# yh-jun/SNR-Aligned_diffSE

Measured on AMD Instinct MI355X. Metric: utterances/sec (4 s @16 kHz, N=30 PC steps) at 1/2/4/8 MI355X; PESQ delta vs ref, higher is better.
Workload: dtype fp16; 1 GPU; C2: B=32 4 s/16 kHz clips per GPU, N=30 PC steps (reverse_diffusion + ald, 60 NFE/utt), OUVE SDE, NCSN++ nf=128, fp16; global_batch=32, per_gpu_batch=32, seq_len=512, parallelism=dp1 (utterance sharding)

## Files before the change

### snr-aligned_diffse_amd/csrc/conv.hip

```cpp
#include "conv_common.h"

#include <algorithm>
#include <type_traits>

using namespace snrse_conv;

namespace {

template <int NWM, int BN>
SNRSE_DEV void block_stats_flush(const ConvParams& p, const float* red, int blk_b, int blk_n0) {
  asm volatile("s_waitcnt lgkmcnt(0)" ::: "memory");
  __builtin_amdgcn_s_barrier();
  const int slot = blockIdx.x & (SNRSE_STAT_SLOTS - 1);
  for (int t = threadIdx.x; t < 2 * BN; t += blockDim.x) {
    float a = 0.f;
#pragma unroll
    for (int w = 0; w < NWM; ++w) a += red[w * 2 * BN + t];
    if (blk_n0 + (t >> 1) < p.Cout)
      unsafeAtomicAdd(&p.stats[stat_idx(blk_b, slot, blk_n0 + (t >> 1), p.Cout) + (t & 1)], (double)a);
  }
}

template <typename TO, int NWM, int BN, bool DEFER = false, int LA = 8>
SNRSE_DEV void epilogue_lds(const ConvParams& p, const f32x4 (&acc)[4][4], int mb, int nb, int lane, float* stage,
// ... 953 lines not shown
                                                 (float*)(smem + 8 * (64 * 68 * 4)), wr, bb, n0, p.W - TW);
}

template <int BM, int BN, typename T, typename TO>
__global__ __launch_bounds__(512) void conv_glds_kernel(ConvParams p) {
  constexpr int WM = BM / 64, WN = BN / 64;
  static_assert(WM * WN == 8, "8 waves");
  constexpr int FM = 4, FN = 4, TM = 64, TN = 64;
  constexpr int STAGES = 3;
  constexpr int A_BYTES = BM * 128, B_BYTES = BN * 128, STAGE = A_BYTES + B_BYTES;
  constexpr int AJ = BM / 64, BJ = BN / 64;
  constexpr int KT = 64;
  extern __shared__ __attribute__((aligned(16))) char smem[];

  const int tid = threadIdx.x, lane = tid & 63;
  const int wid = __builtin_amdgcn_readfirstlane(tid >> 6);
  const int wm = wid / WN, wn = wid % WN;
  const int wg = xcd_block_id(blockIdx.x, gridDim.x);
  const int ks = wg % p.ksplit, tl = wg / p.ksplit;
  const int m0 = (tl / p.ntn) * BM;
  const int n0 = (tl % p.ntn) * BN;

  const int HW = p.H * p.W;
  const int Cin = p.C0 + p.C1;
  const int cblocks = Cin / KT;
  const int nk0 = p.ksize * p.ksize * cblocks;
  const int Csc_all = p.Csc + p.Csc1;
  const int nk = nk0 + (p.sc_src ? Csc_all / KT : 0);
  const int K1 = p.ksize * p.ksize * Cin;
  const int half = p.ksize >> 1;
  const int slot = lane & 7;

  int a_pix[AJ], a_h[AJ], a_w[AJ], a_ch[AJ];
  bool a_ok[AJ];
#pragma unroll
  for (int j = 0; j < AJ; ++j) {
    const int row = (wid * AJ + j) * 8 + (lane >> 3);
    const int m = m0 + row;
    a_ok[j] = m < p.M;
    const int mm = a_ok[j] ? m : 0;
    const int b = mm / HW, rem = mm - b * HW;
    a_h[j] = rem / p.W;
    a_w[j] = rem - a_h[j] * p.W;
    a_pix[j] = mm;
    a_ch[j] = slot ^ (row & 7);
  }

#define SNRSE_ISSUE(KT_, STAGE_)                                                                      \
  do {                                                                                              \
    const int kt_ = (KT_);                                                                          \
    char* sa_ = smem + (STAGE_) * STAGE;                                                            \
    char* sb_ = sa_ + A_BYTES;                                                                      \
    int cs_, cc_, dy_, dx_, wld_, koff_;                                                            \
    const void* abase_;                                                                             \
    long long abytes_;                                                                              \
    const void* wbase_;                                                                             \
    long long wbytes_;                                                                              \
    if (kt_ < nk0) {                                                                                \
      const int tap_ = kt_ / cblocks;                                                               \
      const int c_ = (kt_ - tap_ * cblocks) * KT;                                                   \
      dy_ = tap_ / p.ksize - half;                                                                  \
      dx_ = tap_ - (tap_ / p.ksize) * p.ksize - half;                                               \
      const bool u1_ = c_ >= p.C0;                                                                  \
      abase_ = u1_ ? p.src1 : p.src0;                                                               \
      abytes_ = u1_ ? p.bytes1 : p.bytes0;                                                          \
      cs_ = u1_ ? p.C1 : p.C0;                                                                      \
      cc_ = u1_ ? c_ - p.C0 : c_;                                                                   \
      wbase_ = p.wgt;                                                                               \
      wbytes_ = p.wbytes;                                                                           \
      wld_ = K1;                                                                                    \
      koff_ = tap_ * Cin + c_;                                                                      \
    } else {                                                                                        \
      const int c_ = (kt_ - nk0) * KT;                                                              \
      const bool u1_ = c_ >= p.Csc;                                                                 \
      abase_ = u1_ ? p.sc_src1 : p.sc_src;                                                          \
      abytes_ = u1_ ? p.sc_bytes1 : p.sc_bytes0;                                                    \
      cs_ = u1_ ? p.Csc1 : p.Csc;                                                                   \
      cc_ = u1_ ? c_ - p.Csc : c_;                                                                  \
      dy_ = 0;                                                                                      \
      dx_ = 0;                                                                                      \
      wbase_ = p.sc_wgt;                                                                            \
      wbytes_ = p.sc_wbytes;                                                                        \
      wld_ = Csc_all;                                                                               \
      koff_ = c_;                                                                                   \
    }                                                                                               \
    const __amdgpu_buffer_rsrc_t ra_ = make_rsrc(abase_, abytes_);                                  \
    const __amdgpu_buffer_rsrc_t rb_ = make_rsrc(wbase_, wbytes_);                                  \
    const int shift_ = dy_ * p.W + dx_;                                                             \
    _Pragma("unroll") for (int j = 0; j < AJ; ++j) {                                                \
      const int hh_ = a_h[j] + dy_, ww_ = a_w[j] + dx_;                                             \
      const bool ok_ = a_ok[j] && hh_ >= 0 && hh_ < p.H && ww_ >= 0 && ww_ < p.W;                   \
      const unsigned voff_ =                                                                        \
          ok_ ? (unsigned)(((a_pix[j] + shift_) * cs_ + cc_ + a_ch[j] * 8) * 2) : 0x80000000u;      \
      __builtin_amdgcn_raw_ptr_buffer_load_lds(                                                     \
          ra_, (__attribute__((address_space(3))) void*)(sa_ + (wid * AJ + j) * 1024), 16, voff_, 0, 0, 0); \
    }                                                                                               \
    _Pragma("unroll") for (int j = 0; j < BJ; ++j) {                                                \
      const int row_ = (wid * BJ + j) * 8 + (lane >> 3);                                            \
      const int chk_ = slot ^ (row_ & 7);                                                           \
      const unsigned voff_ = (unsigned)(((n0 + row_) * wld_ + koff_ + chk_ * 8) * 2);               \
      __builtin_amdgcn_raw_ptr_buffer_load_lds(                                                     \
          rb_, (__attribute__((address_space(3))) void*)(sb_ + (wid * BJ + j) * 1024), 16, voff_, 0, 0, 0); \
    }                                                                                               \
  } while (0)

  f32x4 acc[FM][FN];
#pragma unroll
  for (int i = 0; i < FM; ++i)
#pragma unroll
    for (int j = 0; j < FN; ++j) acc[i][j] = f32x4{0.f, 0.f, 0.f, 0.f};

  const int kb = (int)((long long)ks * nk / p.ksplit), ke = (int)((long long)(ks + 1) * nk / p.ksplit);
  SNRSE_ISSUE(kb, 0);
  if (ke - kb > 1) SNRSE_ISSUE(kb + 1, 1);
  const int lrow = lane & 15, lg = lane >> 4;
  int stage = 0;
  for (int kt = kb; kt < ke; ++kt) {
    if (kt + 1 < ke)
      asm volatile("s_waitcnt vmcnt(%0)" ::"n"(AJ + BJ) : "memory");
    else
      asm volatile("s_waitcnt vmcnt(0)" ::: "memory");
    __builtin_amdgcn_s_barrier();
    if (kt + 2 < ke) SNRSE_ISSUE(kt + 2, stage == 0 ? 2 : stage - 1);
    const char* sa = smem + stage * STAGE;
    const char* sb = sa + A_BYTES;
#pragma unroll
    for (int s = 0; s < 2; ++s) {
      u32x4 af[FM], bfr[FN];
#pragma unroll
      for (int i = 0; i < FM; ++i) af[i] = *(const u32x4*)(sa + swz(wm * TM + i * 16 + lrow, 4 * s + lg));
#pragma unroll
      for (int j = 0; j < FN; ++j) bfr[j] = *(const u32x4*)(sb + swz(wn * TN + j * 16 + lrow, 4 * s + lg));
#pragma unroll
      for (int i = 0; i < FM; ++i)
#pragma unroll
        for (int j = 0; j < FN; ++j) acc[i][j] = mfma_chunk<T>(af[i], bfr[j], acc[i][j]);
    }
    stage = stage == STAGES - 1 ? 0 : stage + 1;
  }
#undef SNRSE_ISSUE
  if (p.ksplit > 1) {
    float* const wsp = p.ws + (size_t)ks * p.M * p.Cout;
#pragma unroll
    for (int i = 0; i < FM; ++i)
#pragma unroll
      for (int e = 0; e < 4; ++e) {
        const int m = m0 + wm * TM + i * 16 + lg * 4 + e;
        if (m < p.M) {
#pragma unroll
          for (int j = 0; j < FN; ++j) wsp[(size_t)m * p.Cout + n0 + wn * TN + j * 16 + lrow] = acc[i][j][e];
        }
      }
    return;
  }
  asm volatile("s_waitcnt vmcnt(0) lgkmcnt(0)" ::: "memory");
  __builtin_amdgcn_s_barrier();
  const int b_lo = m0 / HW, b_hi = (min(m0 + BM, p.M) - 1) / HW;
  epilogue_lds<TO, WM, BN, false, sizeof(TO) == 2 ? 8 : 1>(p, acc, m0 + wm * TM, n0 + wn * TN, lane, (float*)(smem + wid * (64 * 68 * 4)),
                           (float*)(smem + 8 * (64 * 68 * 4)), wm, b_lo == b_hi ? b_lo : -1, n0);
}

template <typename TO>
__global__ __launch_bounds__(256) void conv_splitk_finalize(ConvParams p, int ppb) {
  __shared__ float red[16 * 256];
  const int HW = p.H * p.W;
  const int nbi = (HW + ppb - 1) / ppb;
  const int b = blockIdx.x / nbi;
  const int px0 = (blockIdx.x - b * nbi) * ppb, px1 = min(HW, px0 + ppb);
  const int cl = (threadIdx.x & 15) * 8, r0 = threadIdx.x >> 4;
  const int n = blockIdx.y * 128 + cl;
  float add[8], cw[8][4], cb[8], s1[8], s2[8];
#pragma unroll
  for (int k = 0; k < 8; ++k) {
    add[k] = (p.bias ? p.bias[n + k] : 0.f) + (p.temb ? p.temb[(size_t)b * p.temb_stride + n + k] : 0.f);
    s1[k] = 0.f;
    s2[k] = 0.f;
    cb[k] = 0.f;
    cw[k][0] = cw[k][1] = cw[k][2] = cw[k][3] = 0.f;
    if (p.comb_src) {
      cw[k][0] = p.comb_w[(n + k) * 4 + 0];
      cw[k][1] = p.comb_w[(n + k) * 4 + 1];
      cw[k][2] = p.comb_w[(n + k) * 4 + 2];
      cw[k][3] = p.comb_w[(n + k) * 4 + 3];
      cb[k] = p.comb_b[n + k];
    }
  }
  const size_t plane = (size_t)p.M * p.Cout;
  for (int px = px0 + r0; px < px1; px += 16) {
    const size_t m = (size_t)b * HW + px;
    const float* w = p.ws + m * p.Cout + n;
    f32x4 a0 = *(const f32x4*)w, a1 = *(const f32x4*)(w + 4);
    int s = 1;
    for (; s + 4 <= p.ksplit; s += 4) {
      f32x4 q[4][2];
#pragma unroll
      for (int u = 0; u < 4; ++u) {
        q[u][0] = *(const f32x4*)(w + (s + u) * plane);
        q[u][1] = *(const f32x4*)(w + (s + u) * plane + 4);
      }
#pragma unroll
      for (int u = 0; u < 4; ++u) {
        a0 += q[u][0];
        a1 += q[u][1];
      }
    }
    for (; s < p.ksplit; ++s) {
      a0 += *(const f32x4*)(w + s * plane);
      a1 += *(const f32x4*)(w + s * plane + 4);
    }
    float v[8];
#pragma unroll
    for (int k = 0; k < 4; ++k) {
      v[k] = a0[k] + add[k];
      v[4 + k] = a1[k] + add[4 + k];
    }
    if (p.res) {
      if constexpr (sizeof(TO) == 2) {
        epi_residual<TO>(*(const u32x4*)((const TO*)p.res + m * p.res_ld + n), v);
      } else {
        const float* rp = (const float*)p.res + m * p.res_ld + n;
#pragma unroll
        for (int k = 0; k < 8; ++k) v[k] += rp[k];
      }
    }
#pragma unroll
    for (int k = 0; k < 8; ++k) v[k] *= p.out_scale;
    if (p.comb_src) {
      const f32x4 q = *(const f32x4*)(p.comb_src + m * 4);
#pragma unroll
      for (int k = 0; k < 8; ++k) v[k] += q[0] * cw[k][0] + q[1] * cw[k][1] + q[2] * cw[k][2] + q[3] * cw[k][3] + cb[k];
    }
    if constexpr (sizeof(TO) == 2) {
      *(u32x4*)((TO*)p.out + m * p.out_ld + n) = epi_pack<TO>(v);
    } else {
      float* op = (float*)p.out + m * p.out_ld + n;
#pragma unroll
      for (int k = 0; k < 8; ++k) op[k] = v[k];
    }
#pragma unroll
    for (int k = 0; k < 8; ++k) {
      s1[k] += v[k];
      s2[k] = fmaf(v[k], v[k], s2[k]);
    }
  }
  if (p.stats) {
#pragma unroll
    for (int k = 0; k < 8; ++k) {
      red[r0 * 256 + (cl + k) * 2] = s1[k];
      red[r0 * 256 + (cl + k) * 2 + 1] = s2[k];
    }
    __syncthreads();
    const int t = threadIdx.x;
    float a = 0.f;
#pragma unroll
    for (int r = 0; r < 16; ++r) a += red[r * 256 + t];
    unsafeAtomicAdd(&p.stats[stat_idx(b, blockIdx.x & (SNRSE_STAT_SLOTS - 1), blockIdx.y * 128 + (t >> 1), p.Cout) +
                             (t & 1)],
                    (double)a);
  }
}


template <typename T, typename TO, int GNM, int EF, int TW, bool SCD>
__global__ __launch_bounds__(256, 2) void conv_halo5_kernel(ConvParams p) {
  constexpr int TH = 256 / TW, HC = TW + 2;
  constexpr int RW = TH / 4;
  constexpr int HROWS = (TH + 2) * HC;
  constexpr int HJ = (HROWS + 63) / 64;
  constexpr int HALO_BYTES = HROWS * 64;
  constexpr int TAPB = 128 * 64;
  constexpr int SLOT = 3 * TAPB;
  constexpr int KT = 32;
  static_assert(64 * HJ >= HROWS, "halo rows");
  extern __shared__ __attribute__((aligned(16))) char smem[];
  char* const halo = smem;
  char* const ring = smem + HALO_BYTES;
  float* const gnl = (float*)(smem + HALO_BYTES + 2 * SLOT + 1024);

  const int tid = threadIdx.x, lane = tid & 63;
  const int wid = __builtin_amdgcn_readfirstlane(tid >> 6);
#ifdef SNRSE_STAMPS
  constexpr int kStampOff = (HALO_BYTES + 2 * SLOT + 1280) > (4 * (64 * 68 * 4) + 4 * 128 * 2 * 4)
                                ? (HALO_BYTES + 2 * SLOT + 1280) : (4 * (64 * 68 * 4) + 4 * 128 * 2 * 4);
  unsigned long long* const lst = (unsigned long long*)(smem + kStampOff) + wid * 32;
#endif
  SNRSE_STAMP(0);
  const int wg = xcd_block_id(blockIdx.x, gridDim.x);
  const int n0 = (wg % p.ntn) * 128;
  int tile = wg / p.ntn;
  const int ntw = p.W / TW, nth = p.H / TH;
  const int w0 = (tile % ntw) * TW;
  tile /= ntw;
  const int h0 = (tile % nth) * TH;
  const int bb = tile / nth;

  const int Cin = p.C0 + p.C1;
  const int cbm = Cin / KT;
  const int Csc_all = p.Csc + p.Csc1;
  const int cbs = p.sc_src ? Csc_all / KT : 0;
  const int nq = 3 * cbm + cbs;
  const int K1 = 9 * Cin;
  const int hcol = tid & 3;

  int hpix[HJ];
  bool hok[HJ];
#pragma unroll
  for (int j = 0; j < HJ; ++j) {
    const int hr = (tid >> 2) + 64 * j;
    const int hy = hr / HC, hx = hr - (hr / HC) * HC;
    const int ih = h0 + hy - 1, iw = w0 + hx - 1;
    hok[j] = hr < HROWS && ih >= 0 && ih < p.H && iw >= 0 && iw < p.W;
    hpix[j] = (bb * p.H + ih) * p.W + iw;
  }

  u32x4 hv[HJ];
  f32x4 gnv;

#define SNRSE_HALO5_LOADS(BASE_, BYTES_, CS_, CC_)                                                     \
  do {                                                                                              \
    const __amdgpu_buffer_rsrc_t r_ = make_rsrc((BASE_), (BYTES_));                                 \
    const int cs_ = (CS_), cc_ = (CC_) + hcol * 8;                                                  \
    _Pragma("unroll") for (int j = 0; j < HJ; ++j) {                                                \
      const int voff_ = hok[j] ? (hpix[j] * cs_ + cc_) * 2 : (int)0x80000000;                       \
      hv[j] = __builtin_amdgcn_raw_buffer_load_b128(r_, voff_, 0, 0);                               \
    }                                                                                               \
  } while (0)
  auto halo_load = [&](int c) {
    const int ch = c * KT;
    const bool s1 = ch >= p.C0;
    SNRSE_HALO5_LOADS(s1 ? p.src1 : p.src0, s1 ? p.bytes1 : p.bytes0, s1 ? p.C1 : p.C0, s1 ? ch - p.C0 : ch);
    if constexpr (GNM > 0) {
      if (tid < 16) gnv = *(const f32x4*)((tid < 8 ? p.gn_scale : p.gn_shift) + (size_t)bb * Cin + ch + (tid & 7) * 4);
    }
  };
#undef SNRSE_HALO5_LOADS
  auto gn_publish = [&]() {
    if constexpr (GNM > 0) {
      if (tid < 16) {
        f32x4 g = gnv;
        if constexpr (GNM == 2) g *= kNegLog2e;
        *(f32x4*)(gnl + tid * 4) = g;
      }
    }
  };
  auto halo_store = [&](int c) {
    const bool tr = GNM > 0;
    float gsc[8], gsh[8];
    if constexpr (GNM > 0) {
      if (tr) {
        const f32x4 s0 = *(const f32x4*)(gnl + hcol * 8), s1 = *(const f32x4*)(gnl + hcol * 8 + 4);
        const f32x4 t0 = *(const f32x4*)(gnl + 32 + hcol * 8), t1 = *(const f32x4*)(gnl + 32 + hcol * 8 + 4);
#pragma unroll
        for (int i = 0; i < 4; ++i) { gsc[i] = s0[i]; gsc[4 + i] = s1[i]; gsh[i] = t0[i]; gsh[4 + i] = t1[i]; }
      }
    }
#pragma unroll
    for (int j = 0; j < HJ; ++j) {
      const int hr = (tid >> 2) + 64 * j;
      if (j == HJ - 1 && hr >= HROWS) break;
      u32x4 v = hv[j];
      if constexpr (GNM > 0) {
        if (tr) v = gn_xform8<T, GNM>(v, gsc, gsh, hok[j]);
      }
      *(u32x4*)(halo + swz64(hr, hcol)) = v;
    }
  };
  auto dma = [&](int c, int g, int u, char* dst, bool oob = false) {
    const int rl = lane >> 2, sl = lane & 3;
    const unsigned oobm = oob ? 0x80000000u : 0u;
    if (g < 3) {
      const __amdgpu_buffer_rsrc_t r = make_rsrc(p.wgt, p.wbytes);
      const int kb = c * KT;
#pragma unroll
      for (int k = 0; k < 6; ++k) {
        const int ii = wid + 4 * k;
        const int jt = ii >> 3, pc = ii & 7;
        const int row = pc * 16 + rl;
        const unsigned voff = oobm | (unsigned)(((n0 + row) * K1 + (3 * g + jt) * Cin + kb + (sl ^ ((row >> 1) & 3)) * 8) * 2);
        __builtin_amdgcn_raw_ptr_buffer_load_lds(
            r, (__attribute__((address_space(3))) void*)(dst + jt * TAPB + pc * 1024), 16, voff, 0, 0, 0);
      }
    } else {
      const __amdgpu_buffer_rsrc_t r = make_rsrc(p.sc_wgt, p.sc_wbytes);
      const int kb = u * KT;
#pragma unroll
      for (int k = 0; k < 2; ++k) {
        const int pc = wid + 4 * k;
        const int row = pc * 16 + rl;
        const unsigned voff = oobm | (unsigned)(((n0 + row) * Csc_all + kb + (sl ^ ((row >> 1) & 3)) * 8) * 2);
        __builtin_amdgcn_raw_ptr_buffer_load_lds(
            r, (__attribute__((address_space(3))) void*)(dst + pc * 1024), 16, voff, 0, 0, 0);
      }
      const bool one = kb >= p.Csc;
      const __amdgpu_buffer_rsrc_t rx = one ? make_rsrc(p.sc_src1, p.sc_bytes1) : make_rsrc(p.sc_src, p.sc_bytes0);
      const int cs = one ? p.Csc1 : p.Csc, cb = one ? kb - p.Csc : kb;
      const int pix0 = (bb * p.H + h0) * p.W + w0;
#pragma unroll
      for (int k = 0; k < 4; ++k) {
        const int pc = wid + 4 * k;
        const int row = pc * 16 + rl;
        const int pix = pix0 + (row / TW) * p.W + row % TW;
        const unsigned voff = oobm | (unsigned)((pix * cs + cb + (sl ^ ((row >> 1) & 3)) * 8) * 2);
        __builtin_amdgcn_raw_ptr_buffer_load_lds(
            rx, (__attribute__((address_space(3))) void*)(dst + TAPB + pc * 1024), 16, voff, 0, 0, 0);
      }
    }
  };
  f32x4 acc[2][4][4];
#pragma unroll
  for (int h = 0; h < 2; ++h)
#pragma unroll
    for (int i = 0; i < 4; ++i)
#pragma unroll
      for (int j = 0; j < 4; ++j) acc[h][i][j] = f32x4{0.f, 0.f, 0.f, 0.f};
  const int lrow = lane & 15, lg = lane >> 4;
  auto vm_after_dma = [&]() { __builtin_amdgcn_s_waitcnt(0x0f76); };


  if constexpr (SCD) {
    auto nsc = [&](int c) { return (c + 1) * cbs / cbm - c * cbs / cbm; };
    auto kind_of = [](int s, int k, int& su) -> int {
      su = 0;
      if (k >= 3) {
        if (s == 0 || s == 2 || s == 4) return s >> 1;
        su = s <= 3 ? s >> 1 : s - 3;
        return 3;
      }
      if (s < 2) return s;
      if (k == 0) return 2;
      if (k == 1) {
        if (s == 2) return 2;
        return 3;
      }
      if (s == 3) return 2;
      su = s == 2 ? 0 : 1;
      return 3;
    };
    auto m2_pos = [](int k) { return k >= 3 ? 4 : k == 2 ? 3 : 2; };
    halo_load(0);
    dma(0, 0, 0, ring);
    if constexpr (GNM > 0) {
      gn_publish();
      __syncthreads();
    }
    halo_store(0);
    const bool w0g = GNM > 0 && wid == 0;
    bool halo_inflight = false;
    int c = 0, pos = 0, k = nsc(0), ub = 0;
    for (int q = 0; q < nq; ++q) {
      int su;
      const int kind = kind_of(pos, k, su);
      int c2 = c, pos2 = pos + 1, k2 = k, ub2 = ub;
      if (pos2 == 3 + k) { c2 = c + 1; pos2 = 0; ub2 = ub + k; k2 = c2 < cbm ? nsc(c2) : 0; }
      int su2;
      const int kind2 = kind_of(pos2, k2, su2);
      if (halo_inflight) {
        if (w0g) asm volatile("s_waitcnt vmcnt(%0) lgkmcnt(0)" ::"n"(HJ + 1) : "memory");
        else asm volatile("s_waitcnt vmcnt(%0) lgkmcnt(0)" ::"n"(HJ) : "memory");
      } else {
        asm volatile("s_waitcnt vmcnt(0) lgkmcnt(0)" ::: "memory");
      }
      __builtin_amdgcn_s_barrier();
      dma(c2 < cbm ? c2 : 0, kind2, ub2 + su2, ring + ((q + 1) & 1) * SLOT, q + 1 >= nq);
      halo_inflight = false;
      if (kind == 0 && c + 1 < cbm) {
        vm_after_dma();
        halo_load(c + 1);
        halo_inflight = true;
      }
      const char* sl = ring + (q & 1) * SLOT;
      const bool mainph = kind < 3;
      const char* abuf = mainph ? halo : sl + TAPB;
      const int ntap = mainph ? 3 : 1, rs = mainph ? HC : TW;
      for (int jt = 0; jt < ntap; ++jt) {
        const int tp = 3 * kind + jt;
        const int dy = tp / 3 - 1, dx = tp - (tp / 3) * 3 - 1;
        const int arow = mainph ? (wid * RW + dy + 1) * HC + dx + 1 + lrow : wid * RW * TW + lrow;
        const char* sb = sl + jt * TAPB;
        u32x4 af[4], bfr[8];
#pragma unroll
        for (int i = 0; i < 4; ++i) af[i] = *(const u32x4*)(abuf + swz64(arow + (16 * i / TW) * rs + (16 * i) % TW, lg));
#pragma unroll
        for (int j = 0; j < 8; ++j) bfr[j] = *(const u32x4*)(sb + swz64(j * 16 + lrow, lg));
#pragma unroll
        for (int h = 0; h < 2; ++h)
#pragma unroll
          for (int i = 0; i < 4; ++i)
#pragma unroll
            for (int j = 0; j < 4; ++j) acc[h][i][j] = mfma_chunk<T>(af[i], bfr[h * 4 + j], acc[h][i][j]);
      }
      if (c + 1 < cbm) {
        if (kind == 2) {
          gn_publish();
          if (k == 0) {
            asm volatile("s_waitcnt lgkmcnt(0)" ::: "memory");
            __builtin_amdgcn_s_barrier();
            vm_after_dma();
            halo_store(c + 1);
          }
        } else if (kind == 3 && pos == m2_pos(k) + 1) {
          vm_after_dma();
          halo_store(c + 1);
        }
      }
      c = c2; pos = pos2; k = k2; ub = ub2;
    }
  } else {
  halo_load(0);
  dma(0, 0, 0, ring);
  if constexpr (GNM > 0) {
    gn_publish();
    __syncthreads();
  }
  halo_store(0);
  SNRSE_STAMP(1);
  bool halo_inflight = false;
  const bool w0g = GNM > 0 && wid == 0;
  for (int q = 0; q < nq; ++q) {
    const int c = q / 3, t0 = (q - c * 3) * 3;
    const bool first = t0 == 0, last = t0 == 6;
    if (halo_inflight) {
      if (w0g) asm volatile("s_waitcnt vmcnt(%0) lgkmcnt(0)" ::"n"(HJ + 1) : "memory");
      else asm volatile("s_waitcnt vmcnt(%0) lgkmcnt(0)" ::"n"(HJ) : "memory");
    } else {
      asm volatile("s_waitcnt vmcnt(0) lgkmcnt(0)" ::: "memory");
    }
    __builtin_amdgcn_s_barrier();
    SNRSE_STAMP(2 + 2 * (q & 15));
    dma(q + 1 < nq ? (q + 1) / 3 : 0, (q + 1) % 3, 0, ring + ((q + 1) & 1) * SLOT, q + 1 >= nq);
    halo_inflight = false;
    if (first && c + 1 < cbm) {
      vm_after_dma();
      halo_load(c + 1);
      halo_inflight = !last && q + 1 < nq;
    }
    const char* sl = ring + (q & 1) * SLOT;
    for (int jt = 0; jt < 3; ++jt) {
      const int tp = t0 + jt;
      const int dy = tp / 3 - 1, dx = tp - (tp / 3) * 3 - 1;
      const int hbase = (wid * RW + dy + 1) * HC + dx + 1 + lrow;
      const char* sb = sl + jt * TAPB;
      u32x4 af[4], bfr[8];
#pragma unroll
      for (int i = 0; i < 4; ++i) af[i] = *(const u32x4*)(halo + swz64(hbase + (16 * i / TW) * HC + (16 * i) % TW, lg));
#pragma unroll
      for (int j = 0; j < 8; ++j) bfr[j] = *(const u32x4*)(sb + swz64(j * 16 + lrow, lg));
#pragma unroll
      for (int h = 0; h < 2; ++h)
#pragma unroll
        for (int i = 0; i < 4; ++i)
#pragma unroll
          for (int j = 0; j < 4; ++j)
            acc[h][i][j] = mfma_chunk<T>(af[i], bfr[h * 4 + j], acc[h][i][j]);
    }
    SNRSE_STAMP(3 + 2 * (q & 15));
    if (last && c + 1 < cbm) {
      gn_publish();
      asm volatile("s_waitcnt lgkmcnt(0)" ::: "memory");
      __builtin_amdgcn_s_barrier();
      vm_after_dma();
      halo_store(c + 1);
    }
  }
  }
  SNRSE_STAMP(28);
  float add0[16 / sizeof(TO)], add1[16 / sizeof(TO)];
  epi_add<TO, EF>(p, n0, lane, bb, add0);
  epi_add<TO, EF>(p, n0 + 64, lane, bb, add1);
  asm volatile("s_waitcnt vmcnt(0) lgkmcnt(0)" ::: "memory");
  __builtin_amdgcn_s_barrier();
  float* const stage = (float*)(smem + wid * (64 * 68 * 4));
  float* const red = (float*)(smem + 4 * (64 * 68 * 4));
  const int mrow = (bb * p.H + h0 + wid * RW) * p.W + w0;
  constexpr int ELA = sizeof(TO) == 2 ? 8 : 2;
  epilogue_img<TO, 4, 128, true, EF, TW, ELA>(p, acc[0], mrow, n0, lane, stage, red, wid, bb, n0, p.W - TW, add0);
  asm volatile("s_waitcnt lgkmcnt(0)" ::: "memory");
  __builtin_amdgcn_wave_barrier();
  SNRSE_STAMP(26);
  epilogue_img<TO, 4, 128, true, EF, TW, ELA>(p, acc[1], mrow, n0 + 64, lane, stage, red, wid, bb, n0, p.W - TW, add1);
  SNRSE_STAMP(27);
  if (EF < 0 ? p.stats != nullptr : (EF & EF_STATS) != 0) block_stats_flush<4, 128>(p, red, bb, n0);
#ifdef SNRSE_STAMPS
  {
    unsigned long long st_[29];
    if (lane == 0)
      for (int i = 0; i < 29; ++i) st_[i] = lst[i];
    unsigned long long t_end;
    asm volatile("s_waitcnt vmcnt(0)\n\ts_memtime %0\n\ts_waitcnt lgkmcnt(0)" : "=s"(t_end)::"memory");
    unsigned hw, xcc;
    asm volatile("s_getreg_b32 %0, hwreg(HW_REG_HW_ID)" : "=s"(hw));
    asm volatile("s_getreg_b32 %0, hwreg(HW_REG_XCC_ID)" : "=s"(xcc));
    if (lane == 0 && p.stamps) {
      unsigned long long* g = p.stamps + ((size_t)blockIdx.x * 8 + wid) * 32;
      for (int i = 0; i < 29; ++i) g[i] = st_[i];
      g[29] = t_end;
      g[30] = hw;
      g[31] = xcc;
    }
  }
#endif
}


template <auto K, typename... Args>
int launch_dyn_lds(dim3 grid, dim3 block, size_t lds, hipStream_t s, const Args&... args) {
  static const hipError_t attr = hipFuncSetAttribute((const void*)K, hipFuncAttributeMaxDynamicSharedMemorySize, (int)lds);
  SNRSE_RET(attr);
  hipLaunchKernelGGL(K, grid, block, lds, s, args...);
  return (int)hipGetLastError();
}

template <typename TO>
int launch_splitk_finalize(const ConvParams& p, hipStream_t s) {
  const int HW = p.H * p.W, ppb = 64;
  hipLaunchKernelGGL((conv_splitk_finalize<TO>), dim3(p.B * ((HW + ppb - 1) / ppb), p.Cout / 128), dim3(256), 0, s, p,
                     ppb);
  return (int)hipGetLastError();
}

inline int k_tiles(const ConvParams& p, int KT) {
  return p.ksize * p.ksize * ((p.C0 + p.C1) / KT) + (p.sc_src ? (p.Csc + p.Csc1) / KT : 0);
}

inline int stream_output(const snrse_ctx& cx, long long bytes) {
  return cx.epi_nt == 2 ? bytes > ((long long)cx.epi_nt_mb << 20) : cx.epi_nt;
}

template <typename T, typename TO, int GNM, int EF, int TW, bool SCD>
int launch_halo5_ef(ConvParams p, int grid, hipStream_t s) {
  constexpr size_t main_lds = (256 / TW + 2) * (TW + 2) * 64 + 2 * 3 * 128 * 64 + 1024 + 256;
  constexpr size_t epi_lds = 4 * (64 * 68 * 4) + 4 * 128 * 2 * 4;
#ifdef SNRSE_STAMPS
  constexpr size_t lds = (main_lds > epi_lds ? main_lds : epi_lds) + 1024;
#else
  constexpr size_t lds = main_lds > epi_lds ? main_lds : epi_lds;
#endif
  return launch_dyn_lds<conv_halo5_kernel<T, TO, GNM, EF, TW, SCD>>(dim3(grid), dim3(256), lds, s, p);
}

template <typename T, typename TO, int GNM, int TW>
int launch_halo5_gn(ConvParams p, hipStream_t s, snrse_ctx& cx) {
  p.ntn = p.Cout / 128;
  p.epi_nt = stream_output(cx, (long long)p.M * p.out_ld * (long long)sizeof(TO));
  cx.last_epi_nt = p.epi_nt;
  const int tiles = p.B * (p.H / (256 / TW)) * (p.W / TW) * p.ntn;
  const int grid = tiles;
  const bool scd = p.sc_src != nullptr;
  if constexpr (sizeof(TO) == 2 && GNM != 1) {
    if (cx.h5_specialise && p.bias) {
#define SNRSE_H5_EF(F) \
  case (F): return launch_halo5_ef<T, TO, GNM, (F), TW, false>(p, grid, s);
#define SNRSE_H5_EFS(F) \
  case (F): return launch_halo5_ef<T, TO, GNM, (F), TW, true>(p, grid, s);
      if (!scd) {
        switch (epi_flags(p)) {
          SNRSE_H5_EF(EF_TEMB | EF_STATS)
          SNRSE_H5_EF(EF_TEMB | EF_STATS | EF_NT)
          SNRSE_H5_EF(EF_RES | EF_STATS)
          SNRSE_H5_EF(EF_RES | EF_STATS | EF_NT)
          SNRSE_H5_EF(EF_STATS)
          SNRSE_H5_EF(EF_STATS | EF_NT)
          SNRSE_H5_EF(EF_TEMB)
          default: break;
        }
      } else {
        switch (epi_flags(p)) {
          SNRSE_H5_EFS(EF_STATS)
          SNRSE_H5_EFS(EF_STATS | EF_NT)
          SNRSE_H5_EFS(EF_COMB | EF_STATS)
          default: break;
        }
      }
#undef SNRSE_H5_EF
#undef SNRSE_H5_EFS
    }
  }
  return scd ? launch_halo5_ef<T, TO, GNM, EF_RT, TW, true>(p, grid, s)
             : launch_halo5_ef<T, TO, GNM, EF_RT, TW, false>(p, grid, s);
}

template <typename T, typename TO, int TW>
int launch_halo5_tw(ConvParams p, hipStream_t s, snrse_ctx& cx) {
  cx.last_tw = TW;
  if (!p.gn_scale) return launch_halo5_gn<T, TO, 0, TW>(p, s, cx);
  if (!p.gn_act) return launch_halo5_gn<T, TO, 1, TW>(p, s, cx);
  return launch_halo5_gn<T, TO, 2, TW>(p, s, cx);
}

inline bool halo_tile32(const ConvParams& p) { return p.H % 8 == 0 && p.W % 32 == 0; }
inline bool halo_tile64(const ConvParams& p) { return p.H % 4 == 0 && p.W % 64 == 0; }

template <typename T, typename TO>
int launch_halo5(ConvParams p, hipStream_t s, snrse_ctx& cx) {
  if (halo_tile32(p) && cx.h5_tw != 64) return launch_halo5_tw<T, TO, 32>(p, s, cx);
  return launch_halo5_tw<T, TO, 64>(p, s, cx);
}

int choose_ksplit(const ConvParams& p, int tiles, int nk, const snrse_ctx& cx, int min_kt = 4) {
  if (!cx.splitk || !cx.ws || tiles >= cx.splitk_target * 3 / 4) return 1;
  int s = (cx.splitk_target + tiles - 1) / tiles;
  if (s > nk / min_kt) s = nk / min_kt;
  const size_t plane = (size_t)p.M * p.Cout * sizeof(float);
  if ((size_t)s * plane > cx.ws_bytes) s = (int)(cx.ws_bytes / plane);
  return s >= 2 ? s : 1;
}

template <typename T, typename TO, int BM, int BN, int WM, int WN>
int launch_conv(ConvParams p, int npad, hipStream_t s, snrse_ctx& cx) {
  p.ntn = npad / BN;
  const int tiles = ((p.M + BM - 1) / BM) * p.ntn;
  p.ksplit = (sizeof(T) == 4 && BN == 128 && p.Cout % 128 == 0)
                 ? choose_ksplit(p, tiles, k_tiles(p, ConvTraits<T>::KT), cx, 2) : 1;
  p.ws = cx.ws;
  cx.last_ksplit = p.ksplit;
  const size_t lds = (size_t)2 * (BM + BN) * 128;
  hipLaunchKernelGGL((conv_mfma_kernel<T, TO, BM, BN, WM, WN>), dim3(tiles * p.ksplit), dim3(64 * WM * WN), lds, s, p);
  if (p.ksplit == 1) return (int)hipGetLastError();
  SNRSE_LAUNCH_CHECK();
  return launch_splitk_finalize<TO>(p, s);
}

template <int BM, int BN, int WM, int WN>
int launch_x3(ConvParams p, hipStream_t s, snrse_ctx& cx) {
  constexpr size_t main_lds = (size_t)2 * (BM + BN) * 128;
  constexpr size_t epi_lds = (BM / WM == 64 && BN / WN == 64) ? (size_t)WM * WN * 64 * 68 * 4 + WM * BN * 2 * 4 : 0;
  constexpr size_t lds = main_lds > epi_lds ? main_lds : epi_lds;
  p.ntn = (p.Cout + BN - 1) / BN;
  const int tiles = ((p.M + BM - 1) / BM) * p.ntn;
  p.ksplit = BN == 128 ? choose_ksplit(p, tiles, k_tiles(p, SplitBf16Opnd::KT), cx, 2) : 1;
  p.ws = cx.ws;
  cx.last_ksplit = p.ksplit;
  const int rc = launch_dyn_lds<conv_x3_kernel<BM, BN, WM, WN>>(dim3(tiles * p.ksplit), dim3(64 * WM * WN), lds, s, p);
  if (rc || p.ksplit == 1) return rc;
  return launch_splitk_finalize<float>(p, s);
}

template <int GNM, int SPR, int TWV, int EF = EF_RT>
int launch_x3h_ef(ConvParams p, hipStream_t s, int tiles) {
  p.ntn = p.Cout / 128;
  p.ksplit = 1;
  return launch_dyn_lds<conv_x3h_kernel<GNM, SPR, TWV, EF>>(dim3(tiles), dim3(512), X3G<TWV, SPR>::LDS, s, p);
}

template <int GNM, int SPR, int TWV>
int launch_x3h_gn(const ConvParams& p, hipStream_t s, int tiles, bool spec) {
  if constexpr (GNM != 1 && SPR == 2 && TWV == 32) {
    if (spec && p.bias) {
      switch (epi_flags(p)) {
        case EF_TEMB | EF_STATS: return launch_x3h_ef<GNM, SPR, TWV, EF_TEMB | EF_STATS>(p, s, tiles);
        case EF_TEMB | EF_STATS | EF_NT: return launch_x3h_ef<GNM, SPR, TWV, EF_TEMB | EF_STATS | EF_NT>(p, s, tiles);
        case EF_RES | EF_STATS: return launch_x3h_ef<GNM, SPR, TWV, EF_RES | EF_STATS>(p, s, tiles);
        case EF_RES | EF_STATS | EF_NT: return launch_x3h_ef<GNM, SPR, TWV, EF_RES | EF_STATS | EF_NT>(p, s, tiles);
        case EF_STATS: return launch_x3h_ef<GNM, SPR, TWV, EF_STATS>(p, s, tiles);
        case EF_STATS | EF_NT: return launch_x3h_ef<GNM, SPR, TWV, EF_STATS | EF_NT>(p, s, tiles);
        case EF_COMB | EF_STATS: return launch_x3h_ef<GNM, SPR, TWV, EF_COMB | EF_STATS>(p, s, tiles);
        case EF_COMB | EF_STATS | EF_NT: return launch_x3h_ef<GNM, SPR, TWV, EF_COMB | EF_STATS | EF_NT>(p, s, tiles);
        default: break;
      }
    }
  }
  return launch_x3h_ef<GNM, SPR, TWV>(p, s, tiles);
}

template <int SPR, int TWV>
int launch_x3h_spr(const ConvParams& p, hipStream_t s, int tiles, bool spec) {
  if (!p.gn_scale) return launch_x3h_gn<0, SPR, TWV>(p, s, tiles, spec);
  if (!p.gn_act) return launch_x3h_gn<1, SPR, TWV>(p, s, tiles, spec);
  return launch_x3h_gn<2, SPR, TWV>(p, s, tiles, spec);
}

int launch_x3h(const ConvParams& p, hipStream_t s, int tiles, int spread, int tw, bool spec) {
  if (spread == 2 && !(tw == 32 && ((p.C0 + p.C1) / 32) % 2 == 0)) spread = 1;
  if (tw == 32) {
    if (spread == 2) return launch_x3h_spr<2, 32>(p, s, tiles, spec);
    return spread ? launch_x3h_spr<1, 32>(p, s, tiles, spec) : launch_x3h_spr<0, 32>(p, s, tiles, spec);
  }
  return spread ? launch_x3h_spr<1, 64>(p, s, tiles, spec) : launch_x3h_spr<0, 64>(p, s, tiles, spec);
}

template <int BM, int BN, typename T, typename TO>
int launch_glds(ConvParams p, hipStream_t s, snrse_ctx& cx) {
  constexpr size_t lds = (size_t)3 * (BM + BN) * 128;
  p.ntn = p.Cout / BN;
  const int ntm = (p.M + BM - 1) / BM;
  p.ksplit = choose_ksplit(p, ntm * p.ntn, k_tiles(p, 64), cx);
  p.ws = cx.ws;
  cx.last_ksplit = p.ksplit;
  const int rc = launch_dyn_lds<conv_glds_kernel<BM, BN, T, TO>>(dim3(ntm * p.ntn * p.ksplit), dim3(512), lds, s, p);
  if (rc || p.ksplit == 1) return rc;
  return launch_splitk_finalize<TO>(p, s);
}

constexpr int kHaloAuto = 5;

template <typename T, typename TO>
int dispatch_conv(const ConvParams& p, hipStream_t s, snrse_ctx& cx) {
  if (p.Cout >= 64) {
    if (p.Cout % 128 != 0) return SNRSE_EINVAL;
    if constexpr (sizeof(T) == 2) {
      const bool fits = p.bytes0 < 0x7ff00000ll && p.bytes1 < 0x7ff00000ll && p.sc_bytes0 < 0x7ff00000ll &&
                        p.sc_bytes1 < 0x7ff00000ll;
      if (cx.conv_variant != 1 && fits) {
        if (cx.conv_variant != 2 && p.ksize == 3 && halo_tile64(p)) {
          cx.last_kernel = kHaloAuto;
          return launch_halo5<T, TO>(p, s, cx);
        }
        if (p.gn_scale) return SNRSE_EINVAL;
        cx.last_kernel = 2;
        if (p.Cout % 256 == 0) return launch_glds<128, 256, T, TO>(p, s, cx);
        return launch_glds<256, 128, T, TO>(p, s, cx);
      }
    }
    if (p.gn_scale) return SNRSE_EINVAL;
    cx.last_kernel = 1;
    return launch_conv<T, TO, 128, 128, 2, 2>(p, p.Cout, s, cx);
  }
  if constexpr (sizeof(T) == 2 && sizeof(TO) == 4) {
    const bool small = cx.head_small == 2 && (long long)p.B * p.H * p.W <= 16384;
    if (cx.conv_variant != 1 && head_ok(p) && !small) {
      const bool part = cx.head_part != 0 && p.Cout == 4;
      cx.last_kernel = part ? 15 : 10;
      return launch_head(p, s, part, std::is_same_v<T, f16_t>);
    }
    if (cx.conv_variant != 1 && cx.head_small && head_small_ok(p)) {
      cx.last_kernel = 14;
      cx.last_ksplit = 1;
      return launch_head_small(p, s, false, std::is_same_v<T, f16_t>);
    }
  }
  if (p.gn_scale) return SNRSE_EINVAL;
  if (p.Cout > 16) return SNRSE_EINVAL;
  cx.last_kernel = 1;
  return launch_conv<T, TO, 128, 16, 4, 1>(p, 16, s, cx);
}

inline long long x3h_tile_count(const ConvParams& p, int tw) {
  return (long long)p.B * (p.H / (256 / tw)) * ((p.W + tw - 1) / tw) * (p.Cout / 128);
}

int dispatch_x3(const ConvParams& q, hipStream_t stream, snrse_ctx& cx, bool x3h_all) {
  if (x3h_all) {
    cx.last_kernel = 4;
    cx.last_ksplit = 1;
    ConvParams r = q;
    r.epi_nt = cx.x3_nt && stream_output(cx, (long long)q.M * q.out_ld * 4ll) != 0;
    cx.last_epi_nt = r.epi_nt;
    const int tw = (cx.x3_tw != 64 && q.H % 8 == 0 && q.W % 32 == 0) ? 32 : 64;
    cx.last_tw = tw;
    return launch_x3h(r, stream, (int)x3h_tile_count(q, tw), cx.x3_spread, tw, cx.h5_specialise != 0);
  }
  if (q.Cout <= 16 && cx.conv_variant != 1 && head_ok(q, true)) {
    cx.last_kernel = 11;
    cx.last_ksplit = 1;
    return launch_head_x3(q, stream);
  }
  if (q.Cout <= 16 && cx.conv_variant != 1 && cx.head_small && head_small_ok(q)) {
    cx.last_kernel = 14;
    cx.last_ksplit = 1;
    return launch_head_small(q, stream, true);
  }
  if (q.gn_scale) return SNRSE_EINVAL;
  cx.last_kernel = 3;
  if (q.Cout <= 16) return launch_x3<128, 16, 4, 1>(q, stream, cx);
  if (cx.x3_tile == 2) return launch_x3<256, 128, 4, 2>(q, stream, cx);
  if (cx.x3_tile == 3 && q.Cout % 256 == 0) return launch_x3<128, 256, 2, 4>(q, stream, cx);
// ... 117 lines not shown
```

Measured before the change: 13.81 utt/s.

## Interleave weight DMA with MFMAs and precompute buffer offsets in halo conv kernel

The per-step weight and shortcut loads into LDS are no longer issued as one block before the MFMAs. They are split into pairs and interleaved between groups of MFMAs using sched_group_barrier, so the memory issue overlaps tensor-core work. Per-lane buffer offsets are precomputed once and advanced incrementally, and the per-chunk shortcut-count division becomes a running remainder. The halo prefetch is moved after the MFMA block and the GN parameter load is split out. This adds scheduling constraints that could stall if the compiler's ordering conflicts with them, and it changes the vmcnt accounting relative to the halo loads.

```diff
diff --git a/snr-aligned_diffse_amd/csrc/conv.hip b/snr-aligned_diffse_amd/csrc/conv.hip
--- a/snr-aligned_diffse_amd/csrc/conv.hip
+++ b/snr-aligned_diffse_amd/csrc/conv.hip
@@ -1279,6 +1279,31 @@
   const int K1 = 9 * Cin;
   const int hcol = tid & 3;
 
+  const int rl = lane >> 2, swz8 = ((lane & 3) ^ ((rl >> 1) & 3)) * 8;
+  const __amdgpu_buffer_rsrc_t wrsrc = make_rsrc(p.wgt, p.wbytes);
+  const unsigned wlane = (unsigned)(((n0 + wid * 16 + rl) * K1 + swz8) * 2);
+  const unsigned wrow64 = (unsigned)(64 * K1 * 2), wtap = (unsigned)(Cin * 2);
+  using lds_ptr = __attribute__((address_space(3))) void*;
+  auto dma_w = [&](auto k_, unsigned vl, unsigned soff, char* dst) {
+    constexpr int k = decltype(k_)::value;
+    __builtin_amdgcn_raw_ptr_buffer_load_lds(wrsrc, (lds_ptr)(dst + (k >> 1) * TAPB + (wid + 4 * (k & 1)) * 1024), 16,
+                                             vl, soff + (k & 1) * wrow64 + (k >> 1) * wtap, 0, 0);
+  };
+  auto woff = [&](int c, int g) { return (unsigned)((3 * g * Cin + c * KT) * 2); };
+
+  u32x4 hv[HJ];
+  f32x4 gnv;
+  auto gn_load = [&](int c) {
+    if constexpr (GNM > 0) {
+      if (tid < 16)
+        gnv = *(const f32x4*)((tid < 8 ? p.gn_scale : p.gn_shift) + (size_t)bb * Cin + c * KT + (tid & 7) * 4);
+    }
+  };
+
+  static_for<6>([&](auto k) { dma_w(k, wlane, 0u, ring); });
+  gn_load(0);
+  __builtin_amdgcn_sched_barrier(0);
+
   int hpix[HJ];
   bool hok[HJ];
 #pragma unroll
@@ -1289,9 +1314,6 @@
     hok[j] = hr < HROWS && ih >= 0 && ih < p.H && iw >= 0 && iw < p.W;
     hpix[j] = (bb * p.H + ih) * p.W + iw;
   }
-
-  u32x4 hv[HJ];
-  f32x4 gnv;
 
 #define SNRSE_HALO5_LOADS(BASE_, BYTES_, CS_, CC_)                                                     \
   do {                                                                                              \
@@ -1306,9 +1328,6 @@
     const int ch = c * KT;
     const bool s1 = ch >= p.C0;
     SNRSE_HALO5_LOADS(s1 ? p.src1 : p.src0, s1 ? p.bytes1 : p.bytes0, s1 ? p.C1 : p.C0, s1 ? ch - p.C0 : ch);
-    if constexpr (GNM > 0) {
-      if (tid < 16) gnv = *(const f32x4*)((tid < 8 ? p.gn_scale : p.gn_shift) + (size_t)bb * Cin + ch + (tid & 7) * 4);
-    }
   };
 #undef SNRSE_HALO5_LOADS
   auto gn_publish = [&]() {
@@ -1342,47 +1361,6 @@
       *(u32x4*)(halo + swz64(hr, hcol)) = v;
     }
   };
-  auto dma = [&](int c, int g, int u, char* dst, bool oob = false) {
-    const int rl = lane >> 2, sl = lane & 3;
-    const unsigned oobm = oob ? 0x80000000u : 0u;
-    if (g < 3) {
-      const __amdgpu_buffer_rsrc_t r = make_rsrc(p.wgt, p.wbytes);
-      const int kb = c * KT;
-#pragma unroll
-      for (int k = 0; k < 6; ++k) {
-        const int ii = wid + 4 * k;
-        const int jt = ii >> 3, pc = ii & 7;
-        const int row = pc * 16 + rl;
-        const unsigned voff = oobm | (unsigned)(((n0 + row) * K1 + (3 * g + jt) * Cin + kb + (sl ^ ((row >> 1) & 3)) * 8) * 2);
-        __builtin_amdgcn_raw_ptr_buffer_load_lds(
-            r, (__attribute__((address_space(3))) void*)(dst + jt * TAPB + pc * 1024), 16, voff, 0, 0, 0);
-      }
-    } else {
-      const __amdgpu_buffer_rsrc_t r = make_rsrc(p.sc_wgt, p.sc_wbytes);
-      const int kb = u * KT;
-#pragma unroll
-      for (int k = 0; k < 2; ++k) {
-        const int pc = wid + 4 * k;
-        const int row = pc * 16 + rl;
-        const unsigned voff = oobm | (unsigned)(((n0 + row) * Csc_all + kb + (sl ^ ((row >> 1) & 3)) * 8) * 2);
-        __builtin_amdgcn_raw_ptr_buffer_load_lds(
-            r, (__attribute__((address_space(3))) void*)(dst + pc * 1024), 16, voff, 0, 0, 0);
-      }
-      const bool one = kb >= p.Csc;
-      const __amdgpu_buffer_rsrc_t rx = one ? make_rsrc(p.sc_src1, p.sc_bytes1) : make_rsrc(p.sc_src, p.sc_bytes0);
-      const int cs = one ? p.Csc1 : p.Csc, cb = one ? kb - p.Csc : kb;
-      const int pix0 = (bb * p.H + h0) * p.W + w0;
-#pragma unroll
-      for (int k = 0; k < 4; ++k) {
-        const int pc = wid + 4 * k;
-        const int row = pc * 16 + rl;
-        const int pix = pix0 + (row / TW) * p.W + row % TW;
-        const unsigned voff = oobm | (unsigned)((pix * cs + cb + (sl ^ ((row >> 1) & 3)) * 8) * 2);
-        __builtin_amdgcn_raw_ptr_buffer_load_lds(
-            rx, (__attribute__((address_space(3))) void*)(dst + TAPB + pc * 1024), 16, voff, 0, 0, 0);
-      }
-    }
-  };
   f32x4 acc[2][4][4];
 #pragma unroll
   for (int h = 0; h < 2; ++h)
@@ -1395,7 +1373,14 @@
 
 
   if constexpr (SCD) {
-    auto nsc = [&](int c) { return (c + 1) * cbs / cbm - c * cbs / cbm; };
+    const int kq = cbs / cbm, kr = cbs - kq * cbm;
+    int krem = 0;
+    auto nsc_next = [&]() {
+      krem += kr;
+      const bool wrap = krem >= cbm;
+      if (wrap) krem -= cbm;
+      return kq + (wrap ? 1 : 0);
+    };
     auto kind_of = [](int s, int k, int& su) -> int {
       su = 0;
       if (k >= 3) {
@@ -1414,8 +1399,13 @@
       return 3;
     };
     auto m2_pos = [](int k) { return k >= 3 ? 4 : k == 2 ? 3 : 2; };
+    const __amdgpu_buffer_rsrc_t scrsrc = make_rsrc(p.sc_wgt, p.sc_wbytes);
+    const __amdgpu_buffer_rsrc_t xrsrc0 = make_rsrc(p.sc_src, p.sc_bytes0), xrsrc1 = make_rsrc(p.sc_src1, p.sc_bytes1);
+    const unsigned sclane = (unsigned)(((n0 + wid * 16 + rl) * Csc_all + swz8) * 2);
+    const unsigned scrow64 = (unsigned)(64 * Csc_all * 2);
+    const int trow = wid * 16 + rl;
+    const int xpix = (bb * p.H + h0 + trow / TW) * p.W + w0 + trow % TW;
     halo_load(0);
-    dma(0, 0, 0, ring);
     if constexpr (GNM > 0) {
       gn_publish();
       __syncthreads();
@@ -1423,12 +1413,11 @@
     halo_store(0);
     const bool w0g = GNM > 0 && wid == 0;
     bool halo_inflight = false;
-    int c = 0, pos = 0, k = nsc(0), ub = 0;
+    int c = 0, pos = 0, k = nsc_next(), ub = 0;
+    int su, kind = kind_of(0, k, su);
     for (int q = 0; q < nq; ++q) {
-      int su;
-      const int kind = kind_of(pos, k, su);
       int c2 = c, pos2 = pos + 1, k2 = k, ub2 = ub;
-      if (pos2 == 3 + k) { c2 = c + 1; pos2 = 0; ub2 = ub + k; k2 = c2 < cbm ? nsc(c2) : 0; }
+      if (pos2 == 3 + k) { c2 = c + 1; pos2 = 0; ub2 = ub + k; k2 = c2 < cbm ? nsc_next() : 0; }
       int su2;
       const int kind2 = kind_of(pos2, k2, su2);
       if (halo_inflight) {
@@ -1438,33 +1427,73 @@
         asm volatile("s_waitcnt vmcnt(0) lgkmcnt(0)" ::: "memory");
       }
       __builtin_amdgcn_s_barrier();
-      dma(c2 < cbm ? c2 : 0, kind2, ub2 + su2, ring + ((q + 1) & 1) * SLOT, q + 1 >= nq);
-      halo_inflight = false;
-      if (kind == 0 && c + 1 < cbm) {
-        vm_after_dma();
-        halo_load(c + 1);
-        halo_inflight = true;
-      }
+      char* const nx = ring + ((q + 1) & 1) * SLOT;
+      __amdgpu_buffer_rsrc_t Rc, Rn;
+      unsigned Vc, Vn, Sc, Sn, Oc, On, DPn;
+      int DDn;
+      char* Dc = nx + wid * 1024;
+      char* Dn = Dc + TAPB;
+      if (kind2 < 3) {
+        const bool fin = q + 1 >= nq;
+        Rc = Rn = wrsrc;
+        Vc = Vn = fin ? wlane | 0x80000000u : wlane;
+        Sc = fin ? 0u : woff(c2, kind2);
+        Sn = Sc + wtap; DPn = wtap; DDn = TAPB;
+        Oc = On = wrow64;
+      } else {
+        const int kb = (ub2 + su2) * KT;
+        const bool one = kb >= p.Csc;
+        const int cs = one ? p.Csc1 : p.Csc, cb = one ? kb - p.Csc : kb;
+        const unsigned xstep = (unsigned)((64 / TW) * p.W * cs * 2);
+        Rc = scrsrc; Vc = sclane; Sc = (unsigned)(kb * 2); Oc = scrow64;
+        Rn = one ? xrsrc1 : xrsrc0;
+        Vn = (unsigned)((xpix * cs + swz8) * 2);
+        Sn = (unsigned)(cb * 2); On = xstep; DPn = 2 * xstep; DDn = 8192;
+      }
+      auto dma_pair = [&]() {
+        __builtin_amdgcn_raw_ptr_buffer_load_lds(Rc, (lds_ptr)Dc, 16, Vc, Sc, 0, 0);
+        __builtin_amdgcn_raw_ptr_buffer_load_lds(Rc, (lds_ptr)(Dc + 4096), 16, Vc, Sc + Oc, 0, 0);
+        Rc = Rn; Vc = Vn; Sc = Sn; Oc = On; Dc = Dn;
+        Sn += DPn; Dn += DDn;
+      };
       const char* sl = ring + (q & 1) * SLOT;
       const bool mainph = kind < 3;
       const char* abuf = mainph ? halo : sl + TAPB;
       const int ntap = mainph ? 3 : 1, rs = mainph ? HC : TW;
-      for (int jt = 0; jt < ntap; ++jt) {
-        const int tp = 3 * kind + jt;
-        const int dy = tp / 3 - 1, dx = tp - (tp / 3) * 3 - 1;
-        const int arow = mainph ? (wid * RW + dy + 1) * HC + dx + 1 + lrow : wid * RW * TW + lrow;
+      const int arow0 = mainph ? (wid * RW + kind) * HC + lrow : wid * RW * TW + lrow;
+      auto tap_body = [&](int jt, auto gap_) {
+        constexpr bool gap = decltype(gap_)::value;
+        const int arow = arow0 + jt;
         const char* sb = sl + jt * TAPB;
         u32x4 af[4], bfr[8];
 #pragma unroll
         for (int i = 0; i < 4; ++i) af[i] = *(const u32x4*)(abuf + swz64(arow + (16 * i / TW) * rs + (16 * i) % TW, lg));
 #pragma unroll
         for (int j = 0; j < 8; ++j) bfr[j] = *(const u32x4*)(sb + swz64(j * 16 + lrow, lg));
-#pragma unroll
-        for (int h = 0; h < 2; ++h)
-#pragma unroll
-          for (int i = 0; i < 4; ++i)
-#pragma unroll
-            for (int j = 0; j < 4; ++j) acc[h][i][j] = mfma_chunk<T>(af[i], bfr[h * 4 + j], acc[h][i][j]);
+        static_for<32>([&](auto m_) {
+          constexpr int m = decltype(m_)::value, h = m >> 4, i = (m >> 2) & 3, j = m & 3;
+          acc[h][i][j] = mfma_chunk<T>(af[i], bfr[h * 4 + j], acc[h][i][j]);
+          if constexpr (gap && (m & 7) == 7 && m < 24) dma_pair();
+        });
+        if constexpr (gap) {
+#pragma unroll
+          for (int u = 0; u < 3; ++u) {
+            __builtin_amdgcn_sched_group_barrier(0x008, 8, 0);
+            __builtin_amdgcn_sched_group_barrier(0x020, 2, 0);
+          }
+          __builtin_amdgcn_sched_group_barrier(0x008, 8, 0);
+        }
+      };
+      tap_body(0, std::true_type{});
+#pragma nounroll
+      for (int jt = 1; jt < ntap; ++jt) tap_body(jt, std::false_type{});
+      if (kind == 0 && c + 1 < cbm) {
+        vm_after_dma();
+        halo_load(c + 1);
+        gn_load(c + 1);
+        halo_inflight = true;
+      } else {
+        halo_inflight = false;
       }
       if (c + 1 < cbm) {
         if (kind == 2) {
@@ -1480,11 +1509,10 @@
           halo_store(c + 1);
         }
       }
-      c = c2; pos = pos2; k = k2; ub = ub2;
+      c = c2; pos = pos2; k = k2; ub = ub2; kind = kind2; su = su2;
     }
   } else {
   halo_load(0);
-  dma(0, 0, 0, ring);
   if constexpr (GNM > 0) {
     gn_publish();
     __syncthreads();
@@ -1493,9 +1521,11 @@
   SNRSE_STAMP(1);
   bool halo_inflight = false;
   const bool w0g = GNM > 0 && wid == 0;
+  int c = 0, g = 0;
+  unsigned soff = woff(0, 1);
+  const unsigned soff_g = 3 * wtap, soff_c = (unsigned)(2 * KT) - 6 * wtap;
   for (int q = 0; q < nq; ++q) {
-    const int c = q / 3, t0 = (q - c * 3) * 3;
-    const bool first = t0 == 0, last = t0 == 6;
+    const bool first = g == 0, last = g == 2;
     if (halo_inflight) {
       if (w0g) asm volatile("s_waitcnt vmcnt(%0) lgkmcnt(0)" ::"n"(HJ + 1) : "memory");
       else asm volatile("s_waitcnt vmcnt(%0) lgkmcnt(0)" ::"n"(HJ) : "memory");
@@ -1504,33 +1534,47 @@
     }
     __builtin_amdgcn_s_barrier();
     SNRSE_STAMP(2 + 2 * (q & 15));
-    dma(q + 1 < nq ? (q + 1) / 3 : 0, (q + 1) % 3, 0, ring + ((q + 1) & 1) * SLOT, q + 1 >= nq);
-    halo_inflight = false;
+    const bool fin = q + 1 >= nq;
+    const unsigned vl = fin ? wlane | 0x80000000u : wlane, so = fin ? 0u : soff;
+    char* const nx = ring + ((q + 1) & 1) * SLOT;
+    const char* sl = ring + (q & 1) * SLOT;
+    const int hrow = (wid * RW + g) * HC + lrow;
+    static_for<3>([&](auto jt_) {
+      constexpr int jt = decltype(jt_)::value;
+      const int hbase = hrow + jt;
+      const char* sb = sl + jt * TAPB;
+      u32x4 af[4], bfr[8];
+#pragma unroll
+      for (int i = 0; i < 4; ++i) af[i] = *(const u32x4*)(halo + swz64(hbase + (16 * i / TW) * HC + (16 * i) % TW, lg));
+#pragma unroll
+      for (int j = 0; j < 8; ++j) bfr[j] = *(const u32x4*)(sb + swz64(j * 16 + lrow, lg));
+      static_for<32>([&](auto m_) {
+        constexpr int m = decltype(m_)::value, h = m >> 4, i = (m >> 2) & 3, j = m & 3;
+        acc[h][i][j] = mfma_chunk<T>(af[i], bfr[h * 4 + j], acc[h][i][j]);
+        if constexpr (jt < 2 && (m & 7) == 7 && m < 24)
+          dma_w(std::integral_constant<int, 3 * jt + (m >> 3)>{}, vl, so, nx);
+      });
+    });
+    static_assert(sizeof(T) == 2, "one MFMA per mfma_chunk");
+#pragma unroll
+    for (int t = 0; t < 2; ++t) {
+#pragma unroll
+      for (int u = 0; u < 3; ++u) {
+        __builtin_amdgcn_sched_group_barrier(0x008, 8, 0);
+        __builtin_amdgcn_sched_group_barrier(0x020, 1, 0);
+      }
+      __builtin_amdgcn_sched_group_barrier(0x008, 8, 0);
+    }
+    __builtin_amdgcn_sched_group_barrier(0x008, 32, 0);
+    SNRSE_STAMP(3 + 2 * (q & 15));
     if (first && c + 1 < cbm) {
       vm_after_dma();
       halo_load(c + 1);
-      halo_inflight = !last && q + 1 < nq;
-    }
-    const char* sl = ring + (q & 1) * SLOT;
-    for (int jt = 0; jt < 3; ++jt) {
-      const int tp = t0 + jt;
-      const int dy = tp / 3 - 1, dx = tp - (tp / 3) * 3 - 1;
-      const int hbase = (wid * RW + dy + 1) * HC + dx + 1 + lrow;
-      const char* sb = sl + jt * TAPB;
-      u32x4 af[4], bfr[8];
-#pragma unroll
-      for (int i = 0; i < 4; ++i) af[i] = *(const u32x4*)(halo + swz64(hbase + (16 * i / TW) * HC + (16 * i) % TW, lg));
-#pragma unroll
-      for (int j = 0; j < 8; ++j) bfr[j] = *(const u32x4*)(sb + swz64(j * 16 + lrow, lg));
-#pragma unroll
-      for (int h = 0; h < 2; ++h)
-#pragma unroll
-        for (int i = 0; i < 4; ++i)
-#pragma unroll
-          for (int j = 0; j < 4; ++j)
-            acc[h][i][j] = mfma_chunk<T>(af[i], bfr[h * 4 + j], acc[h][i][j]);
-    }
-    SNRSE_STAMP(3 + 2 * (q & 15));
+      gn_load(c + 1);
+      halo_inflight = true;
+    } else {
+      halo_inflight = false;
+    }
     if (last && c + 1 < cbm) {
       gn_publish();
       asm volatile("s_waitcnt lgkmcnt(0)" ::: "memory");
@@ -1538,6 +1582,9 @@
       vm_after_dma();
       halo_store(c + 1);
     }
+    soff += g == 1 ? soff_c : soff_g;
+    if (last) { g = 0; ++c; }
+    else ++g;
   }
   }
   SNRSE_STAMP(28);
```

Result: faster. 14.14 utt/s (median of 6 runs) (+2.4%).
